# ruihuang1124/CAFE-MPC

Hardware: AMD Instinct MI355X
Metric: DDP iterations/sec, Mini-Cheetah WB N=200, batch=4096; 1/2/4/8 GPU (higher is better)
Workload: dtype f64

## Files before the change

cafe-mpc_amd/csrc/sweep.hpp:

```cpp
#pragma once
#include <cstddef>
#include <limits>
#include <type_traits>
#include "hs_types.hpp"
#include "hs_mfma.hpp"

namespace hs {

constexpr int SW_NT = 256;
constexpr int SW_SET_WB = 0, SW_SET_HKD = 1;
constexpr int SW_N = 36;
constexpr int SW_PRE = 20;
#ifndef SW_UNROLL_N
#define SW_UNROLL_N 4
#endif
#define HS_STR_(x) #x
#define HS_UNROLL_N(n) _Pragma(HS_STR_(unroll n))
#ifndef SW_LDLT_NB
#define SW_LDLT_NB ((M <= 12 || sizeof(R) == 4) ? 2 : 1)
#endif
#ifndef SW_MINB
#define SW_MINB 2
#endif
#ifndef SW_LDLT_WDW
#define SW_LDLT_WDW 1
#endif
#ifndef SW_OVERLAP_LDLT
#define SW_OVERLAP_LDLT 1
#endif

template <int N, int M, int PY, class R = double> struct SweepLdsT {
    static constexpr int LDN = N + 1, LDM = (M > PY ? M : PY) + 1, PYd = PY > 0 ? PY : 1;
    static constexpr int AR = rec_arows(N), LDA = AR + 1, A0 = N - AR;
    R H[LDN * N], A[LDA * N], HA[LDN * N];
    R B[LDA * M], HB[LDN * M];
    R Qux[LDM * N];
    union { R K[LDM * N]; R lC[PY > 0 ? LDM * N : 1]; };
    R C[PY > 0 ? LDM * N : 1], D[PY > 0 ? LDM * M : 1];
    union { R LQ[LDM * M]; R lD[PY > 0 ? LDM * M : 1]; };
    R lyy[PY > 0 ? LDM * PY : 1], Quu[LDM * M];
    R G[N], Gn[N], Qx[N], Qu[M], dU[M], ly[PYd], def[N];
};
template <int N, int M, int PY, class R = double> struct LinLdsT {
    static constexpr int AR = rec_arows(N), A0 = N - AR;
    R A[2][AR * N], Q[2][N * N], B[2][AR * M], K[2][M * N], U[2][M * M], v[2][256];
    R dx[N], dxn[N], du[M];
};
struct SweepCtl { double dV1, dV2, xfer[SW_N]; unsigned long long t_last; int ok; };
constexpr size_t sw_max(size_t a, size_t b) { return a > b ? a : b; }
template <class R> constexpr size_t sweep_bytes_wb() { return sw_max(sw_max(sizeof(SweepLdsT<36, 12, 12, R>), sizeof(LinLdsT<36, 12, 12, R>)), sw_max(sizeof(SweepLdsT<12, 12, 0, R>), sizeof(LinLdsT<12, 12, 0, R>))); }
template <class R> constexpr size_t sweep_bytes_hkd() { return sw_max(sw_max(sizeof(SweepLdsT<24, 24, 0, R>), sizeof(LinLdsT<24, 24, 0, R>)), sw_max(sizeof(SweepLdsT<12, 12, 0, R>), sizeof(LinLdsT<12, 12, 0, R>))); }
template <class R, int SET> struct SweepLdsRaw { R raw[(SET == 0 ? sweep_bytes_wb<R>() : sweep_bytes_hkd<R>()) / sizeof(R)]; SweepCtl c; };
using SweepLds = SweepLdsRaw<double, 0>;
using SweepLdsHkd = SweepLdsRaw<double, 1>;
using SweepLds32 = SweepLdsRaw<float, 1>;

#define CM(M, i, j, ld) (M)[(i) + (ld) * (j)]

#if defined(SW_PROF) && !defined(HS_HOST_EMU)
__device__ unsigned long long g_sw_prof[48];
#define SW_STAMP(i) { if (blockIdx.x == 0 && threadIdx.x == 0) { unsigned long long t_ = clock64(); atomicAdd(&g_sw_prof[i], t_ - SWC.t_last); SWC.t_last = t_; } }
#define SW_STAMP0() { if (blockIdx.x == 0 && threadIdx.x == 0) SWC.t_last = clock64(); }
#define SW_WSTAMP(p) { if (blockIdx.x == 0 && (tid & 63) == 0) atomicAdd(&g_sw_prof[16 + 4 * (p) + (tid >> 6)], clock64() - SWC.t_last); }
#else
#define SW_WSTAMP(p)
#define SW_STAMP(i)
#define SW_STAMP0()
#endif

#ifdef HS_HOST_EMU
#define SW_PRE_DECL static R pre_all_[SW_NT][SW_PRE];
#define PRE(r) pre_all_[tid][r]
#else
#define SW_PRE_DECL R pre_[SW_PRE];
#define PRE(r) pre_[r]
#endif

#ifndef HS_HOST_EMU
template <int CTRL> HD double dpp_quad(double v) {
    const int lo = __builtin_amdgcn_mov_dpp(__double2loint(v), CTRL, 0xf, 0xf, true), hi = __builtin_amdgcn_mov_dpp(__double2hiint(v), CTRL, 0xf, 0xf, true);
    return __hiloint2double(hi, lo);
}
HD double quad_sum(double v) { v += dpp_quad<0xB1>(v); v += dpp_quad<0x4E>(v); return v; }
template <int CTRL> HD float dpp_quad(float v) { return __int_as_float(__builtin_amdgcn_mov_dpp(__float_as_int(v), CTRL, 0xf, 0xf, true)); }
HD float quad_sum(float v) { v += dpp_quad<0xB1>(v); v += dpp_quad<0x4E>(v); return v; }
#endif
#ifdef HS_HOST_EMU
#define SW_QS 1
#define SW_QUAD_ROWS(CNT, PARTIAL, FINISH) if (tid < (CNT)) { const int o = tid; R p_[4]; R p2_[4]; for (int part = 0; part < 4; part++) { R partial = 0; R partial2 = 0; PARTIAL p_[part] = partial; p2_[part] = partial2; } \
    const R total = (p_[0] + p_[1]) + (p_[2] + p_[3]); const R total2 = (p2_[0] + p2_[1]) + (p2_[2] + p2_[3]); (void)total2; FINISH }
#else
#define SW_QS 4
#define SW_QUAD_ROWS(CNT, PARTIAL, FINISH) if ((tid >> 2) < (CNT)) { const int o = tid >> 2; const int part = tid & 3; R partial = 0; R partial2 = 0; PARTIAL \
    const R total = quad_sum(partial); const R total2 = quad_sum(partial2); (void)total2; if (part == 0) FINISH }
#endif

template <int M, int LD, class R, int PART>
HD void ldlt_parts(int tid, const R* A, R diag_add, R* NI, R* Lw, int* iw, int* ok, R* W1 = nullptr, R* W2 = nullptr) {
    const R TOL = R(1.0) / std::numeric_limits<R>::max();
#ifdef HS_HOST_EMU
    if (PART == 2) return;
    if (tid == 0) {
        R m[M * M]; int tr[M]; int sign = 0; (void)Lw; (void)iw;
        for (int j = 0; j < M; j++) for (int i = 0; i < M; i++) m[i + M * j] = A[i + LD * j] + (i == j ? diag_add : 0.0);
        auto Mx = [&](int i, int j) -> R& { return m[i + M * j]; };
        R temp[M];
        for (int k = 0; k < M; k++) {
            int big = k; R best = std::fabs(Mx(k, k));
            for (int i = k + 1; i < M; i++) if (std::fabs(Mx(i, i)) > best) { best = std::fabs(Mx(i, i)); big = i; }
            tr[k] = big;
            if (k != big) {
                for (int j = 0; j < k; j++) { const R t = Mx(k, j); Mx(k, j) = Mx(big, j); Mx(big, j) = t; }
                for (int i = big + 1; i < M; i++) { const R t = Mx(i, k); Mx(i, k) = Mx(i, big); Mx(i, big) = t; }
                { const R t = Mx(k, k); Mx(k, k) = Mx(big, big); Mx(big, big) = t; }
                for (int i = k + 1; i < big; i++) { const R t = Mx(i, k); Mx(i, k) = Mx(big, i); Mx(big, i) = t; }
            }
            for (int j = 0; j < k; j++) temp[j] = Mx(j, j) * Mx(k, j);
            { R s = 0; for (int j = 0; j < k; j++) s += Mx(k, j) * temp[j]; Mx(k, k) -= s; }
            for (int i = k + 1; i < M; i++) { R t = 0; for (int j = 0; j < k; j++) t += Mx(i, j) * temp[j]; Mx(i, k) -= t; }
            const R akk = Mx(k, k); const bool valid = std::fabs(akk) > 0.0;
            if (valid) for (int i = k + 1; i < M; i++) Mx(i, k) /= akk;
            if (sign == 1) { if (akk < 0) sign = 2; } else if (sign == -1) { if (akk > 0) sign = 2; } else if (sign == 0) { if (akk > 0) sign = 1; else if (akk < 0) sign = -1; }
        }
        if (!(sign == 1 || sign == 0)) *ok = 0;
        for (int c = 0; c < M; c++) {
            R x[M]; for (int i = 0; i < M; i++) x[i] = (i == c) ? 1.0 : 0.0;
            for (int k = 0; k < M; k++) if (tr[k] != k) { const R t = x[k]; x[k] = x[tr[k]]; x[tr[k]] = t; }
            for (int i = 0; i < M; i++) { R s = x[i]; for (int j = 0; j < i; j++) s -= Mx(i, j) * x[j]; x[i] = s; }
            for (int i = 0; i < M; i++) { const R d = Mx(i, i); x[i] = (std::fabs(d) > TOL) ? x[i] / d : 0.0; }
            for (int i = M - 1; i >= 0; i--) { R s = x[i]; for (int j = i + 1; j < M; j++) s -= Mx(j, i) * x[j]; x[i] = s; }
            for (int k = M - 1; k >= 0; k--) if (tr[k] != k) { const R t = x[k]; x[k] = x[tr[k]]; x[tr[k]] = t; }
            for (int i = 0; i < M; i++) NI[i + LD * c] = -x[i];
        }
    }
#else
    static_assert(M <= 32, "one row per lane");
#if defined(SW_PROF)
#define SW_LSTAMP(i) { if (blockIdx.x == 0 && tid == 0) { const unsigned long long t_ = clock64(); atomicAdd(&g_sw_prof[i], t_ - tl_); tl_ = t_; } }
#else
#define SW_LSTAMP(i)
#endif
    {
#if defined(SW_PROF)
        unsigned long long tl_ = clock64();
#endif
        const bool act = tid < M; const int me = act ? tid : M - 1;
        if (PART != 2) {
        R dg[M];
        _Pragma("unroll") for (int j = 0; j < M; j++) dg[j] = fabs(A[j + LD * j] + diag_add);
        const R mine = fabs(A[me + LD * me] + diag_add);
        int rank = 0; bool tie = false;
        _Pragma("unroll") for (int j = 0; j < M; j++) { const bool eq = (dg[j] == mine) && (j != me); rank += (dg[j] > mine || (eq && j < me)) ? 1 : 0; tie = tie || eq; }
        if (__builtin_amdgcn_ballot_w64(tie && act) == 0ull) { if (act) iw[rank] = me; }
        else {
            int gt = 0, ge = 0;
            _Pragma("unroll") for (int j = 0; j < M; j++) { gt += (dg[j] > mine) ? 1 : 0; ge += (dg[j] >= mine) ? 1 : 0; }
            int ixp = me; if (!act) { gt = M; ge = M; }
            _Pragma("unroll") for (int k = 0; k < M; k++) {
                const unsigned long long at = __builtin_amdgcn_ballot_w64(tid >= k && gt <= k && k < ge);
                const int big = (int)__builtin_ctzll(at);
                if (big != k) {
                    const int ik = __builtin_amdgcn_readlane(ixp, k), gk = __builtin_amdgcn_readlane(gt, k), ek = __builtin_amdgcn_readlane(ge, k);
                    const int ib = __builtin_amdgcn_readlane(ixp, big), gb = __builtin_amdgcn_readlane(gt, big), eb = __builtin_amdgcn_readlane(ge, big);
                    ixp = (tid == k) ? ib : ((tid == big) ? ik : ixp); gt = (tid == k) ? gb : ((tid == big) ? gk : gt); ge = (tid == k) ? eb : ((tid == big) ? ek : ge);
                }
            }
            if (act) iw[tid] = ixp;
        }
        __builtin_amdgcn_fence(__ATOMIC_RELEASE, "wavefront"); __builtin_amdgcn_wave_barrier(); __builtin_amdgcn_fence(__ATOMIC_ACQUIRE, "wavefront");
        SW_LSTAMP(9)
        }
        int pv[M]; int myrank = 0;
        _Pragma("unroll") for (int k = 0; k < M; k++) { pv[k] = iw[k]; myrank = (pv[k] == me) ? k : myrank; }
        if (PART != 2) {
        const int prow = iw[me];
        R arow[M];
        _Pragma("unroll") for (int j = 0; j < M; j++) { const int r = prow > pv[j] ? prow : pv[j], c = prow > pv[j] ? pv[j] : prow; arow[j] = A[r + LD * c] + ((j == me) ? diag_add : 0.0); }
        SW_LSTAMP(10)
        bool anyneg = false;
        _Pragma("unroll") for (int j = 0; j < M; j++) {
            const R d = hs_readlane(arow[j], j);
            R rd = hs_rcp(d); rd = rd * (R(2.0) - d * rd); rd = rd * (R(2.0) - d * rd);
            rd = (fabs(d) > TOL) ? rd : 0.0;
            anyneg = anyneg || (d < 0.0);
            const R lij = (fabs(d) > 0.0) ? arow[j] * rd : arow[j];
            if (M <= 12) { if (act && me >= j) Lw[me * M + j] = (me == j) ? rd : lij; }
            else if (act) { if (me > j) Lw[me * M + j] = lij; else if (me == j) Lw[j * M + j] = rd; }
            _Pragma("unroll") for (int k = j + 1; k < M; k++) arow[k] -= lij * hs_readlane(arow[j], k);
        }
        SW_LSTAMP(11)
        if (tid == 0 && anyneg) *ok = 0;
        }
        if (PART == 1) return;
        __builtin_amdgcn_fence(__ATOMIC_RELEASE, "wavefront"); __builtin_amdgcn_wave_barrier(); __builtin_amdgcn_fence(__ATOMIC_ACQUIRE, "wavefront");
        constexpr int NB = SW_LDLT_NB;
        R y[M], lr[NB][M];
        if (NB == 1) { lr[0][0] = 0.0; }
        _Pragma("unroll") for (int k = 0; k < M; k++) {
            if (NB == 2) { if (k + 1 < M) { _Pragma("unroll") for (int j = 0; j <= k; j++) lr[(k + 1) % NB][j] = Lw[(k + 1) * M + j]; } }
            else { _Pragma("unroll") for (int j = 0; j < k; j++) lr[0][j] = Lw[k * M + j]; }
            HS_CBAR();
            R sacc = (k == myrank) ? 1.0 : 0.0;
            _Pragma("unroll") for (int j = 0; j < k; j++) sacc -= lr[k % NB][j] * y[j];
            HS_PIN(sacc);
            y[k] = sacc;
        }
        SW_LSTAMP(12)
#if SW_LDLT_WDW
        if (PART == 2 && sizeof(R) == 8) {
            if (act) { _Pragma("unroll") for (int k = 0; k < M; k++) { W1[k + M * me] = y[k]; W2[k + M * me] = -(y[k] * Lw[k * M + k]); } }
            __builtin_amdgcn_fence(__ATOMIC_RELEASE, "wavefront"); __builtin_amdgcn_wave_barrier(); __builtin_amdgcn_fence(__ATOMIC_ACQUIRE, "wavefront");
            constexpr int TMq = (M + 15) / 16;
            MTileT<R> td[TMq * TMq];
            _Pragma("unroll") for (int t = 0; t < TMq * TMq; t++) td[t] = MTileT<R>{NI, LD, nullptr, 0, 16 * (t % TMq), 16 * (t / TMq), M, M, W1, M, W2, M, M, true, nullptr, 0, nullptr, 0, 0};
            mfma_tiles<TMq * TMq, (M + 3) / 4 * 4, 0, R>(tid, td);
            SW_LSTAMP(13)
            return;
        }
#endif
        _Pragma("unroll") for (int k = 0; k < M; k++) y[k] = y[k] * Lw[k * M + k];
        _Pragma("unroll") for (int k = M - 1; k >= 0; k--) {
            if (NB == 2) { if (k > 0) { _Pragma("unroll") for (int j = k; j < M; j++) lr[(k - 1) % NB][j] = Lw[j * M + (k - 1)]; } }
            else { _Pragma("unroll") for (int j = k + 1; j < M; j++) lr[0][j] = Lw[j * M + k]; }
            HS_CBAR();
            R sacc = y[k];
            _Pragma("unroll") for (int j = k + 1; j < M; j++) sacc -= lr[k % NB][j] * y[j];
            HS_PIN(sacc);
            y[k] = sacc;
        }
        if (act) { _Pragma("unroll") for (int k = 0; k < M; k++) NI[pv[k] + LD * me] = -y[k]; }
        SW_LSTAMP(13)
    }
#endif
}
template <int M, int LD, class R>
HD void ldlt_inverse_w(const R* A, R diag_add, R* NI, R* Lw, int* iw, int* ok) {
    HS_WPHASE(ldlt_parts<M, LD, R, 0>(tid, A, diag_add, NI, Lw, iw, ok);)
}
template <int NT, class TD, class TS> HD void ld_mat(int tid, TD* dst, int ldd, const TS* src, int rows, int cols) {
    const int i = tid % rows, j0 = tid / rows, js = NT / rows;
    if (j0 < js) for (int j = j0; j < cols; j += js) dst[i + ldd * j] = src[i + rows * j];
}
template <int NT, class TD, class TS> HD void st_mat(int tid, TD* dst, const TS* src, int lds_, int rows, int cols) {
    const int i = tid % rows, j0 = tid / rows, js = NT / rows;
    if (j0 < js) for (int j = j0; j < cols; j += js) dst[i + rows * j] = src[i + lds_ * j];
}

#define SW_RICCATI_FETCH(kk_, k_) { \
    const HS_GLOBAL R* rec_ = grec + (kk_) * (size_t)RL::size + tid; \
    _Pragma("unroll") for (int r = 0; r < RL::rounds; r++) if (r < RL::rA || r >= RL::rA + RL::rQ) PRE(r) = rec_[NT * r];      \
    PRE(RL::rounds) = (tid < N + M + PY) ? rec_[RL::oLx] : (tid < 2 * N + M + PY) ? (R)gDefect[((size_t)b * (h + 1) + (k_) + 1) * N + tid - N - M - PY] : R(0.0); }
#define SW_RICCATI_FETCH_LXX(kk_) { \
    const HS_GLOBAL R* rec_ = grec + (kk_) * (size_t)RL::size + tid; \
    _Pragma("unroll") for (int r = RL::rA; r < RL::rA + RL::rQ; r++) PRE(r) = rec_[NT * r]; }
#define SW_RICCATI_LXX() { \
    _Pragma("unroll") for (int r = 0; r < RL::rQ; r++) { const int e = tid + NT * r; if (e < N * N) S.H[(e % N) + LDN * (e / N)] += PRE(RL::rA + r); } }
#define SW_RICCATI_COMMIT() { \
    constexpr int PYd = PY > 0 ? PY : 1; \
    _Pragma("unroll") for (int r = 0; r < RL::rA; r++) { const int e = tid + NT * r; if (e < AR * N) S.A[(e % AR) + LDA * (e / AR)] = PRE(r); } \
    _Pragma("unroll") for (int r = 0; r < RL::rB; r++) { const int e = tid + NT * r; if (e < AR * M) S.B[(e % AR) + LDA * (e / AR)] = PRE(RL::rA + RL::rQ + r); } \
    _Pragma("unroll") for (int r = 0; r < RL::rC; r++) { const int e = tid + NT * r; if (e < PY * N) S.C[(e % PYd) + LDM * (e / PYd)] = PRE(RL::rA + RL::rQ + RL::rB + r); } \
    _Pragma("unroll") for (int r = 0; r < RL::rD; r++) { const int e = tid + NT * r; if (e < PY * M) S.D[(e % PYd) + LDM * (e / PYd)] = PRE(RL::rA + RL::rQ + RL::rB + RL::rC + r); } \
    _Pragma("unroll") for (int r = 0; r < RL::rLuu; r++) { const int e = tid + NT * r; if (e < M * M) S.Quu[(e % M) + LDM * (e / M)] = PRE(RL::rA + RL::rQ + RL::rB + RL::rC + RL::rD + r); } \
    _Pragma("unroll") for (int r = 0; r < RL::rLyy; r++) { const int e = tid + NT * r; if (e < PY * PY) S.lyy[(e % PYd) + LDM * (e / PYd)] = PRE(RL::rA + RL::rQ + RL::rB + RL::rC + RL::rD + RL::rLuu + r); } \
    if (tid < N) S.Qx[tid] = PRE(RL::rounds); else if (tid < N + M) S.Qu[tid - N] = PRE(RL::rounds); else if (tid < N + M + PY) S.ly[tid - N - M] = PRE(RL::rounds); \
    else if (tid < 2 * N + M + PY) S.def[tid - N - M - PY] = PRE(RL::rounds); }

template <class R> HD const HS_GLOBAL R* rec_of(const PhaseDev& P);
template <> HD const HS_GLOBAL double* rec_of<double>(const PhaseDev& P) { return P.rec; }
template <> HD const HS_GLOBAL float* rec_of<float>(const PhaseDev& P) { return P.rec32; }

template <class E> HD constexpr int deal_order(int n, int ix) {
    int c = 0;
    for (int e = 0; e < n; e++) if (!E::edge(e)) { if (c == ix) return e; c++; }
    for (int e = 0; e < n; e++) if (E::edge(e)) { if (c == ix) return e; c++; }
    return ix;
}
template <int W, int N, int M, int PY, class R, int DEAL = 0>
HD void sweep_tiles1(SweepLdsT<N, M, PY, R>& S, int lane, R dt) {
    constexpr int LDN = SweepLdsT<N, M, PY, R>::LDN, LDM = SweepLdsT<N, M, PY, R>::LDM, AR = SweepLdsT<N, M, PY, R>::AR, LDA = SweepLdsT<N, M, PY, R>::LDA, A0 = SweepLdsT<N, M, PY, R>::A0;
    constexpr int TN = (N + 15) / 16, TM = (M + 15) / 16, TP = (PY + 15) / 16, TPd = TP > 0 ? TP : 1;
    constexpr int t1 = TN * TN, t2 = t1 + TN * TM, t3 = t2 + TP * TN, t4 = t3 + TP * TM;
    constexpr bool WBT = (DEAL == 0 && t4 == 16 && t3 == 15);
    constexpr int nA = t1 + (t3 - t2), nB = (t2 - t1) + (t4 - t3);
    constexpr int NTL = DEAL == 1 ? (W == 0 ? nB : (nA - (W - 1) + 2) / 3) : WBT ? (W == 0 ? 5 : W == 3 ? 3 : 4) : (t4 - W + 3) / 4;
    if (NTL <= 0) return;
    MTileT<R> td[NTL > 0 ? NTL : 1];
    _Pragma("unroll") for (int q = 0; q < NTL; q++) {
        struct E1 { static constexpr bool edge(int e) { return e < t1 ? mfma_edge_tile<R>(N, N, 16 * (e % TN), 16 * (e / TN)) : mfma_edge_tile<R>(PY, N, 16 * ((e - t1) % TPd), 16 * ((e - t1) / TPd)); } };
        const int ix = DEAL == 1 && W > 0 ? deal_order<E1>(nA, (W - 1) + 3 * q) : (W - 1) + 3 * q;
        const int t = DEAL == 1 ? (W == 0 ? (q < t2 - t1 ? t1 + q : t3 + (q - (t2 - t1))) : (ix < t1 ? ix : t2 + (ix - t1))) : (WBT && W == 0 && q == 4) ? 15 : W + 4 * q;
        if (t < t1) { td[q] = MTileT<R>{S.HA, LDN, nullptr, 0, 16 * (t % TN), 16 * (t / TN), N, N, S.H + LDN * A0, LDN, S.A, LDA, AR, false, nullptr, 0, nullptr, 0, 0};
                      if (A0 > 0) { td[q].T = S.H; td[q].ldt = LDN; td[q].tmode = 1; td[q].tsplit = A0; td[q].tscale = dt; } }
        else if (t < t2) td[q] = MTileT<R>{S.HB, LDN, nullptr, 0, 16 * ((t - t1) % TN), 16 * ((t - t1) / TN), N, M, S.H + LDN * A0, LDN, S.B, LDA, AR, false, nullptr, 0, nullptr, 0, 0};
        else if (t < t3) td[q] = MTileT<R>{S.lC, LDM, nullptr, 0, 16 * ((t - t2) % TPd), 16 * ((t - t2) / TPd), PY, N, S.lyy, LDM, S.C, LDM, PY, false, nullptr, 0, nullptr, 0, 0};
        else td[q] = MTileT<R>{S.lD, LDM, nullptr, 0, 16 * ((t - t3) % TPd), 16 * ((t - t3) / TPd), PY, M, S.lyy, LDM, S.D, LDM, PY, false, nullptr, 0, nullptr, 0, 0};
    }
    mfma_tiles<(NTL > 0 ? NTL : 1), ((AR > PY ? AR : PY) + 3) / 4 * 4, 0, R>(lane, td);
}
template <int W, int N, int M, int PY, class R, int DEAL = 0>
HD void sweep_tiles2(SweepLdsT<N, M, PY, R>& S, int lane, R reg, R dt) {
    constexpr int LDN = SweepLdsT<N, M, PY, R>::LDN, LDM = SweepLdsT<N, M, PY, R>::LDM, AR = SweepLdsT<N, M, PY, R>::AR, LDA = SweepLdsT<N, M, PY, R>::LDA, A0 = SweepLdsT<N, M, PY, R>::A0;
    constexpr int TN = (N + 15) / 16, TM = (M + 15) / 16;
    constexpr int t1 = TN * (TN + 1) / 2, t2 = t1 + TM * TN, t3 = t2 + TM * TM;
    constexpr int NTL = DEAL == 0 ? (t3 - W + 3) / 4 : DEAL == 2 ? (t3 - t2 - W + 3) / 4 : (W == 0 ? t3 - t2 : (t2 - (W - 1) + 2) / 3);
    if (NTL <= 0) return;
    MTileT<R> td[NTL > 0 ? NTL : 1];
    _Pragma("unroll") for (int q = 0; q < NTL; q++) {
        struct E2 { static constexpr bool edge(int e) {
            if (e < t1) { int c = 0; for (int jj = 0; jj < TN; jj++) for (int ii = 0; ii <= jj; ii++) { if (c == e) return mfma_edge_tile<R>(N, N, 16 * ii, 16 * jj); c++; } return false; }
            return mfma_edge_tile<R>(M, N, 16 * ((e - t1) % TM), 16 * ((e - t1) / TM)); } };
        const int t = DEAL == 0 ? W + 4 * q : DEAL == 2 ? t2 + W + 4 * q : (W == 0 ? t2 + q : deal_order<E2>(t2, (W - 1) + 3 * q));
        int bi = 0, bj = 0;
        { int c = 0; for (int jj = 0; jj < TN; jj++) for (int ii = 0; ii <= jj; ii++) { if (c == t) { bi = ii; bj = jj; } c++; } }
        if (t < t1) { td[q] = MTileT<R>{S.H, LDN, nullptr, 0, 16 * bi, 16 * bj, N, N, S.A, LDA, S.HA + A0, LDN, AR, true, S.C, LDM, S.lC, LDM, PY}; if (bi == bj) td[q].dadd = reg; else td[q].mirror = true;
                      if (A0 > 0) { td[q].T = S.HA; td[q].ldt = LDN; td[q].tmode = 2; td[q].tsplit = A0; td[q].tscale = dt; } }
        else if (t < t2) td[q] = MTileT<R>{S.Qux, LDM, nullptr, 0, 16 * ((t - t1) % TM), 16 * ((t - t1) / TM), M, N, S.B, LDA, S.HA + A0, LDN, AR, true, S.D, LDM, S.lC, LDM, PY};
        else { td[q] = MTileT<R>{S.Quu, LDM, S.Quu, LDM, 16 * ((t - t2) % TM), 16 * ((t - t2) / TM), M, M, S.B, LDA, S.HB + A0, LDN, AR, true, S.D, LDM, S.lD, LDM, PY}; if ((t - t2) % TM == (t - t2) / TM) td[q].dadd = reg; }
    }
    mfma_tiles<(NTL > 0 ? NTL : 1), (AR + 3) / 4 * 4, (PY + 3) / 4 * 4, R>(lane, td);
}

template <int W, int N, int M, int PY, class R>
HD void sweep_tiles3(SweepLdsT<N, M, PY, R>& S, int lane) {
    constexpr int LDN = SweepLdsT<N, M, PY, R>::LDN, LDM = SweepLdsT<N, M, PY, R>::LDM;
    constexpr int TN = (N + 15) / 16;
    constexpr int NTL = (TN * TN - W + 3) / 4;
    if (NTL <= 0) return;
    MTileT<R> td[NTL > 0 ? NTL : 1];
    _Pragma("unroll") for (int q = 0; q < NTL; q++) {
        struct E3 { static constexpr bool edge(int e) { return mfma_edge_tile<R>(N, N, 16 * (e % TN), 16 * (e / TN)); } };
        const int t = deal_order<E3>(TN * TN, W + 4 * q);
        td[q] = MTileT<R>{S.H, LDN, S.H, LDN, 16 * (t % TN), 16 * (t / TN), N, N, S.Qux, LDM, S.K, LDM, M, true, nullptr, 0, nullptr, 0, 0};
    }
    mfma_tiles<(NTL > 0 ? NTL : 1), (M + 3) / 4 * 4, 0, R>(lane, td);
}

template <int W, int N, int M, int PY, class R>
HD void sweep_tilesK(SweepLdsT<N, M, PY, R>& S, int lane) {
    constexpr int LDM = SweepLdsT<N, M, PY, R>::LDM;
    constexpr int TN = (N + 15) / 16, TM = (M + 15) / 16;
    constexpr int NTL = (TM * TN - W + 3) / 4;
    if (NTL <= 0) return;
    MTileT<R> td[NTL > 0 ? NTL : 1];
    _Pragma("unroll") for (int q = 0; q < NTL; q++) {
        const int t = W + 4 * q;
        td[q] = MTileT<R>{S.K, LDM, nullptr, 0, 16 * (t % TM), 16 * (t / TM), M, N, S.LQ, LDM, S.Qux, LDM, M, false, nullptr, 0, nullptr, 0, 0};
    }
    mfma_tiles<(NTL > 0 ? NTL : 1), (M + 3) / 4 * 4, 0, R>(lane, td);
}

template <int NT, int N, int M, int PY, class R, class LDS>
HD bool riccati_phase(LDS& SS, const PhaseDev& P, int b, R reg) {
    using RL = RecLayout<N, M, PY>; using ST = SweepLdsT<N, M, PY, R>;
    static_assert(NT == 256 && RL::rounds + 1 <= SW_PRE && N <= SW_N && 2 * N + M + PY <= NT && 64 + M <= NT - N - 1 - M && N <= 64 && M <= 64, "sweep limits");
    constexpr bool WBS = (N == 36 && M == 12 && PY == 12);
    constexpr bool OVL = SW_OVERLAP_LDLT != 0;
    constexpr int GN0 = WBS ? 64 : 0, G0 = WBS ? 64 : NT - N, DV0 = WBS ? 64 + N : NT - N - 1, DU0 = WBS ? 64 + N + 1 : NT - N - 1 - M;
    constexpr int LDN = ST::LDN, LDM = ST::LDM, AR = ST::AR, LDA = ST::LDA, A0 = ST::A0;
    static_assert(sizeof(ST) <= sizeof(SS.raw), "the view fits the raw LDS block of its model set");
    ST& S = *reinterpret_cast<ST*>(SS.raw); SweepCtl& SWC = SS.c;
    constexpr int TN = (N + 15) / 16, TM = (M + 15) / 16, TP = (PY + 15) / 16;
    const int h = P.h; const R dtR = (R)P.dt;
    const auto grec = rec_of<R>(P); const auto gDefect = P.Defect; const auto gQu = P.Qu; const auto gQuu = P.Quu; const auto gQux = P.Qux;
    const auto gK = P.K; const auto gdU = P.dU; const auto gG = P.G;
    SW_PRE_DECL
    HS_PHASE(NT, { const int i = tid % N, j0 = tid / N; if (j0 < NT / N) for (int j = j0; j < N; j += NT / N) CM(S.H, i, j, LDN) += P.Phixx[(size_t)b * N * N + i + N * j]; }
             if (tid < N) { const R g = SWC.xfer[tid] + P.Phix[(size_t)b * N + tid]; S.G[tid] = g; gG[((size_t)b * (h + 1) + h) * N + tid] = g; }
             if (tid == 0) { SWC.ok = 1; }
             SW_RICCATI_FETCH((size_t)b * h + (h - 1), h - 1) SW_RICCATI_FETCH_LXX((size_t)b * h + (h - 1)))
    for (int k = h - 1; k >= 0; k--) {
        const size_t kk = (size_t)b * h + k;
        SW_STAMP0()
        HS_PHASE_L(NT, SW_RICCATI_COMMIT() if (k > 0) SW_RICCATI_FETCH(kk - 1, k - 1))
        SW_STAMP(0)
        HS_PHASE_L(NT, {
            const int w = tid >> 6, lane = tid & 63;
            if constexpr (OVL && M > 12) {
            switch (w) { case 0: sweep_tiles1<0, N, M, PY, R>(S, lane, dtR); break; case 1: sweep_tiles1<1, N, M, PY, R>(S, lane, dtR); break;
                         case 2: sweep_tiles1<2, N, M, PY, R>(S, lane, dtR); break; default: sweep_tiles1<3, N, M, PY, R>(S, lane, dtR); }
            } else if constexpr (OVL) {
            switch (w) { case 0: sweep_tiles1<0, N, M, PY, R, 1>(S, lane, dtR);
#ifndef HS_HOST_EMU
                                 __builtin_amdgcn_fence(__ATOMIC_RELEASE, "wavefront"); __builtin_amdgcn_wave_barrier(); __builtin_amdgcn_fence(__ATOMIC_ACQUIRE, "wavefront");
#endif
                                 sweep_tiles2<0, N, M, PY, R, 1>(S, lane, reg, dtR); break;
                         case 1: sweep_tiles1<1, N, M, PY, R, 1>(S, lane, dtR); break;
                         case 2: sweep_tiles1<2, N, M, PY, R, 1>(S, lane, dtR); break; default: sweep_tiles1<3, N, M, PY, R, 1>(S, lane, dtR); }
            } else {
            switch (w) { case 0: sweep_tiles1<0, N, M, PY, R>(S, lane, dtR); break; case 1: sweep_tiles1<1, N, M, PY, R>(S, lane, dtR); break;
                         case 2: sweep_tiles1<2, N, M, PY, R>(S, lane, dtR); break; default: sweep_tiles1<3, N, M, PY, R>(S, lane, dtR); }
            }
            if (tid >= GN0 && tid < GN0 + N) { const int i = tid - GN0; R s = S.G[i]; _Pragma("unroll 6") for (int j = 0; j < N; j++) s += CM(S.H, i, j, LDN) * S.def[j]; S.Gn[i] = s; }
            SW_WSTAMP(0)
        })
        if constexpr (OVL && M > 12) {
            HS_PHASE_L(NT, { const int w = tid >> 6, lane = tid & 63;
                switch (w) { case 0: sweep_tiles2<0, N, M, PY, R, 2>(S, lane, reg, dtR); break; case 1: sweep_tiles2<1, N, M, PY, R, 2>(S, lane, reg, dtR); break;
                             case 2: sweep_tiles2<2, N, M, PY, R, 2>(S, lane, reg, dtR); break; default: sweep_tiles2<3, N, M, PY, R, 2>(S, lane, reg, dtR); } })
        }
        SW_STAMP(1)
        if constexpr (OVL) {
        HS_PHASE_L(NT, {
            const int w = tid >> 6, lane = tid & 63;
            switch (w) { case 0: break; case 1: sweep_tiles2<1, N, M, PY, R, 1>(S, lane, reg, dtR); break;
                         case 2: sweep_tiles2<2, N, M, PY, R, 1>(S, lane, reg, dtR); break; default: sweep_tiles2<3, N, M, PY, R, 1>(S, lane, reg, dtR); }
            if (tid >= 128 && tid < 128 + N) {
                const int i = tid - 128; R s = 0;
                if (A0 > 0) s = (i < A0) ? S.Gn[i] : dtR * S.Gn[i - A0];
                _Pragma("unroll 6") for (int t = 0; t < AR; t++) s += CM(S.A, t, i, LDA) * S.Gn[A0 + t];
                if (PY > 0) { _Pragma("unroll 6") for (int t = 0; t < PY; t++) s += CM(S.C, t, i, LDM) * S.ly[t]; }
                S.Qx[i] += s;
            } else if (tid >= 192 && tid < 192 + M) {
                const int a = tid - 192; R s = 0;
                _Pragma("unroll 6") for (int t = 0; t < AR; t++) s += CM(S.B, t, a, LDA) * S.Gn[A0 + t];
                if (PY > 0) { _Pragma("unroll 6") for (int t = 0; t < PY; t++) s += CM(S.D, t, a, LDM) * S.ly[t]; }
                S.Qu[a] += s;
            }
            if (w == 0) ldlt_parts<M, LDM, R, 1>(lane, S.Quu, R(-1e-9), S.LQ, S.HB, reinterpret_cast<int*>(S.HB + M * M), &SWC.ok);
            SW_WSTAMP(1)
        })
        SW_STAMP(2)
        HS_PHASE_L(NT,
            if (tid < 64) ldlt_parts<M, LDM, R, 2>(tid, S.Quu, R(-1e-9), S.LQ, S.HB, reinterpret_cast<int*>(S.HB + M * M), &SWC.ok, S.HA, S.A);
            else for (int e = tid - 64; e < TN * 256; e += NT - 64) {
                const int i = 16 * (e >> 8) + (e & 15), j = 16 * (e >> 8) + ((e >> 4) & 15);
                if (i < j && j < N) { const R s = (CM(S.H, i, j, LDN) + CM(S.H, j, i, LDN)) / 2; CM(S.H, i, j, LDN) = s; CM(S.H, j, i, LDN) = s; }
            })
        SW_STAMP(5)
        } else {
        HS_PHASE_L(NT, {
            const int w = tid >> 6, lane = tid & 63;
            switch (w) { case 0: sweep_tiles2<0, N, M, PY, R>(S, lane, reg, dtR); break; case 1: sweep_tiles2<1, N, M, PY, R>(S, lane, reg, dtR); break;
                         case 2: sweep_tiles2<2, N, M, PY, R>(S, lane, reg, dtR); break; default: sweep_tiles2<3, N, M, PY, R>(S, lane, reg, dtR); }
            if (tid >= 128 && tid < 128 + N) {
                const int i = tid - 128; R s = 0;
                if (A0 > 0) s = (i < A0) ? S.Gn[i] : dtR * S.Gn[i - A0];
                _Pragma("unroll 6") for (int t = 0; t < AR; t++) s += CM(S.A, t, i, LDA) * S.Gn[A0 + t];
                if (PY > 0) { _Pragma("unroll 6") for (int t = 0; t < PY; t++) s += CM(S.C, t, i, LDM) * S.ly[t]; }
                S.Qx[i] += s;
            } else if (tid >= 192 && tid < 192 + M) {
                const int a = tid - 192; R s = 0;
                _Pragma("unroll 6") for (int t = 0; t < AR; t++) s += CM(S.B, t, a, LDA) * S.Gn[A0 + t];
                if (PY > 0) { _Pragma("unroll 6") for (int t = 0; t < PY; t++) s += CM(S.D, t, a, LDM) * S.ly[t]; }
                S.Qu[a] += s;
            }
            SW_WSTAMP(1)
        })
        SW_STAMP(2)
        HS_PHASE_L(NT, if (tid < M) gQu[kk * M + tid] = S.Qu[tid];
                   st_mat<NT>(tid, gQuu + kk * M * M, S.Quu, LDM, M, M); st_mat<NT>(tid, gQux + kk * M * N, S.Qux, LDM, M, N);)
        SW_STAMP(3)
        ldlt_inverse_w<M, LDM, R>(S.Quu, R(-1e-9), S.LQ, S.HA, reinterpret_cast<int*>(S.HB), &SWC.ok);
        SW_STAMP(4)
        HS_PHASE_L(NT,
            if (tid >= 64) for (int e = tid - 64; e < N * N; e += NT - 64) {
                const int i = e % N, j = e / N;
                if (i < j) {
                    const R s = (i / 16 == j / 16) ? (CM(S.H, i, j, LDN) + CM(S.H, j, i, LDN)) / 2 : CM(S.H, i, j, LDN);
                    CM(S.H, i, j, LDN) = s; CM(S.H, j, i, LDN) = s;
                }
            })
        SW_STAMP(5)
        }
        if (!SWC.ok) return false;
        SW_STAMP(6)
        HS_PHASE_L(NT,
            { const int w = tid >> 6, lane = tid & 63;
              switch (w) { case 0: sweep_tilesK<0, N, M, PY, R>(S, lane); break; case 1: sweep_tilesK<1, N, M, PY, R>(S, lane); break;
                           case 2: sweep_tilesK<2, N, M, PY, R>(S, lane); break; default: sweep_tilesK<3, N, M, PY, R>(S, lane); } }
            if (tid >= NT - M) { const int i = tid - (NT - M); R s = 0; _Pragma("unroll") for (int t = 0; t < M; t++) s += CM(S.LQ, i, t, LDM) * S.Qu[t]; S.dU[i] = s; }
            SW_RICCATI_LXX() if (k > 0) SW_RICCATI_FETCH_LXX(kk - 1) SW_WSTAMP(2))
        HS_PHASE_L(NT,
            { const int w = tid >> 6, lane = tid & 63;
              switch (w) { case 0: sweep_tiles3<0, N, M, PY, R>(S, lane); break; case 1: sweep_tiles3<1, N, M, PY, R>(S, lane); break;
                           case 2: sweep_tiles3<2, N, M, PY, R>(S, lane); break; default: sweep_tiles3<3, N, M, PY, R>(S, lane); } }
            if constexpr (!WBS && M > 12) {
                constexpr int CH = (M + 3) / 4;
                SW_QUAD_ROWS(N, { _Pragma("unroll") for (int jj = 0; jj < CH; jj++) { const int t = part * CH + jj; if (t < M) partial += CM(S.Qux, t, o, LDM) * S.dU[t]; } },
                             { const R s = S.Qx[o] + total; S.G[o] = s; gG[((size_t)b * (h + 1) + k) * N + o] = s; })
            }
            if ((WBS || M <= 12) && tid >= G0 && tid < G0 + N) { const int i = tid - G0; R s = S.Qx[i]; _Pragma("unroll") for (int t = 0; t < M; t++) s += CM(S.Qux, t, i, LDM) * S.dU[t]; S.G[i] = s; gG[((size_t)b * (h + 1) + k) * N + i] = s; }
            else if (tid == DV0) { R dVk = 0; _Pragma("unroll") for (int t = 0; t < M; t++) dVk -= S.Qu[t] * S.dU[t]; SWC.dV1 -= dVk; SWC.dV2 += dVk; }
            else if (tid >= DU0 && tid < DU0 + M) { const int a = tid - DU0; gdU[kk * M + a] = S.dU[a]; } SW_WSTAMP(3))
        SW_STAMP(7)
        if constexpr (OVL) {
        HS_PHASE_L(NT, st_mat<NT>(tid, gK + kk * M * N, S.K, LDM, M, N); if (tid < M) gQu[kk * M + tid] = S.Qu[tid];
                   st_mat<NT>(tid, gQuu + kk * M * M, S.Quu, LDM, M, M); st_mat<NT>(tid, gQux + kk * M * N, S.Qux, LDM, M, N);)
        } else {
        HS_PHASE_L(NT, st_mat<NT>(tid, gK + kk * M * N, S.K, LDM, M, N);)
        }
        SW_STAMP(8)
    }
    HS_PHASE(NT, if (tid < N) S.def[tid] = gDefect[((size_t)b * (h + 1)) * N + tid];)
    HS_PHASE(NT, if (tid < N) { R s = S.G[tid]; for (int j = 0; j < N; j++) s += CM(S.H, tid, j, LDN) * S.def[j]; S.Gn[tid] = s; })
    HS_PHASE(NT, if (tid < N) { SWC.xfer[tid] = S.Gn[tid]; gG[((size_t)b * (h + 1)) * N + tid] = S.Gn[tid]; }
             st_mat<NT>(tid, P.H0 + (size_t)b * N * N, S.H, LDN, N, N);)
    return true;
}

template <int NT, class R, int SET, class LDS>
HD bool riccati_sweep(LDS& S, const PhaseDev* ph, int nph, int b, R reg) {
    HS_PHASE(NT, if (tid == 0) { S.c.dV1 = 0.0; S.c.dV2 = 0.0; })
    for (int i = nph - 1; i >= 0; i--) {
        const PhaseDev& P = ph[i];
        const int n = P.n;
        if (i == nph - 1) {
            HS_PHASE(NT, for (int e = tid; e < (n + 1) * n; e += NT) S.raw[e] = 0.0; if (tid < n) S.c.xfer[tid] = 0.0;)
        } else {
            const int nn = P.next_n, ldh = nn + 1;
            R* Hn = S.raw;
            R* Px = S.raw + (n + 1) * n;
            R* HP = S.raw + 2 * (n + 1) * n;
            const auto* Pxg = P.Px + (size_t)b * nn * n;
            R gnew = 0.0;
            HS_PHASE(NT, for (int e = tid; e < nn * n; e += NT) Px[e] = Pxg[e];)
            HS_PHASE(NT,
                for (int e = tid; e < nn * n; e += NT) { const int r = e % nn, c = e / nn; R s = 0; for (int t = 0; t < nn; t++) s += Hn[r + ldh * t] * Px[t + nn * c]; HP[e] = s; }
                if (tid >= NT - n) { const int i2 = tid - (NT - n); R s = 0; for (int t = 0; t < nn; t++) s += Px[t + nn * i2] * S.c.xfer[t]; S.raw[3 * (n + 1) * n + i2] = s; })
            (void)gnew;
            HS_PHASE(NT,
                for (int e = tid; e < n * n; e += NT) { const int r = e % n, c = e / n; R s = 0; for (int t = 0; t < nn; t++) s += Px[t + nn * r] * HP[t + nn * c]; S.raw[r + (n + 1) * c] = s; }
                if (tid >= NT - n) S.c.xfer[tid - (NT - n)] = S.raw[3 * (n + 1) * n + tid - (NT - n)];)
        }
        bool ok;
        if constexpr (SET == SW_SET_WB) {
            if (P.model == HSDDP_MODEL_WB) ok = riccati_phase<NT, 36, 12, 12, R>(S, P, b, reg); else ok = riccati_phase<NT, 12, 12, 0, R>(S, P, b, reg);
        } else {
            if (P.model == HSDDP_MODEL_SRB) ok = riccati_phase<NT, 12, 12, 0, R>(S, P, b, reg); else ok = riccati_phase<NT, 24, 24, 0, R>(S, P, b, reg);
        }
        if (!ok) return false;
    }
    return true;
}

#define SW_LIN_FETCH(kk_, k_) { \
    const HS_GLOBAL R* rec_ = grec + (kk_) * (size_t)RL::size + tid; \
    _Pragma("unroll") for (int r = 0; r < RL::rA; r++) PRE(r) = rec_[RL::oA + NT * r]; \
    _Pragma("unroll") for (int r = 0; r < RL::rQ; r++) PRE(RL::rA + r) = rec_[RL::oLxx + NT * r]; \
    _Pragma("unroll") for (int r = 0; r < RL::rB; r++) PRE(RL::rA + RL::rQ + r) = rec_[RL::oB + NT * r]; \
    _Pragma("unroll") for (int r = 0; r < rK; r++) { const int e = tid + NT * r; PRE(RL::rA + RL::rQ + RL::rB + r) = (e < M * N) ? (R)gK[(kk_) * M * N + e] : R(0.0); } \
    _Pragma("unroll") for (int r = 0; r < RL::rLuu; r++) PRE(RL::rA + RL::rQ + RL::rB + rK + r) = rec_[RL::oLuu + NT * r]; \
    PRE(RL::rA + RL::rQ + RL::rB + rK + RL::rLuu) = (tid < N + M) ? rec_[RL::oLx] : (tid < N + 2 * M) ? (R)gdU[(kk_) * M + tid - N - M] \
            : (tid < 2 * N + 2 * M) ? (R)gDefect[((size_t)b * (h + 1) + (k_) + 1) * N + tid - N - 2 * M] : R(0.0); }
#define SW_LIN_COMMIT(p_) { \
    R* A_ = S.A[p_]; R* Q_ = S.Q[p_]; R* B_ = S.B[p_]; R* K_ = S.K[p_]; R* U_ = S.U[p_]; R* v_ = S.v[p_]; \
    _Pragma("unroll") for (int r = 0; r < RL::rA; r++) { const int e = tid + NT * r; if (e < AR * N) A_[e] = PRE(r); } \
    _Pragma("unroll") for (int r = 0; r < RL::rQ; r++) { const int e = tid + NT * r; if (e < N * N) Q_[e] = PRE(RL::rA + r); } \
    _Pragma("unroll") for (int r = 0; r < RL::rB; r++) { const int e = tid + NT * r; if (e < AR * M) B_[e] = PRE(RL::rA + RL::rQ + r); } \
    _Pragma("unroll") for (int r = 0; r < rK; r++) { const int e = tid + NT * r; if (e < N * M) K_[e] = PRE(RL::rA + RL::rQ + RL::rB + r); } \
    _Pragma("unroll") for (int r = 0; r < RL::rLuu; r++) { const int e = tid + NT * r; if (e < M * M) U_[e] = PRE(RL::rA + RL::rQ + RL::rB + rK + r); } \
    { const R w_ = PRE(RL::rA + RL::rQ + RL::rB + rK + RL::rLuu); \
      if (tid < N) v_[tid] = w_; else if (tid < N + M) v_[64 + tid - N] = w_; \
      else if (tid < N + 2 * M) v_[128 + tid - N - M] = w_; else if (tid < 2 * N + 2 * M) v_[192 + tid - N - 2 * M] = w_; } }

template <int NT, int N, int M, int PY, class R, class LDS>
HD void linear_phase(LDS& SS, const PhaseDev& P, int b, R eps) {
    using RL = RecLayout<N, M, PY>; using ST = LinLdsT<N, M, PY, R>;
    constexpr int rK = rec_rnd(M * N) / 256, AR = ST::AR, A0 = ST::A0;
    static_assert(RL::rA + RL::rQ + RL::rB + rK + RL::rLuu + 1 <= SW_PRE && 2 * N + 2 * M <= NT && 4 * N <= 192 && 4 * M <= NT && 192 + M <= NT && N <= 64 && M <= 64, "prefetch registers / lane maps");
    const R dtR = (R)P.dt;
    static_assert(offsetof(ST, dx) >= 2 * NT * sizeof(R), "the partial-sum scratch must not reach dx");
    static_assert(sizeof(ST) <= sizeof(SS.raw), "the view fits the raw LDS block of its model set");
    ST& S = *reinterpret_cast<ST*>(SS.raw); SweepCtl& SWC = SS.c;
    const int h = P.h;
    const auto grec = rec_of<R>(P); const auto gDefect = P.Defect; const auto gK = P.K; const auto gdU = P.dU; const auto gdX = P.dX; const auto gKdX = P.KdX;
    SW_PRE_DECL
#ifdef HS_HOST_EMU
    static R acc1_all_[NT], acc2_all_[NT];
    for (int t = 0; t < NT; t++) { acc1_all_[t] = 0.0; acc2_all_[t] = 0.0; }
#define ACC1 acc1_all_[tid]
#define ACC2 acc2_all_[tid]
#else
    R acc1_ = 0.0, acc2_ = 0.0;
#define ACC1 acc1_
#define ACC2 acc2_
#endif
    HS_PHASE(NT, if (tid < N) { R v = SWC.xfer[tid] + eps * gDefect[((size_t)b * (h + 1)) * N + tid]; S.dx[tid] = v; gdX[((size_t)b * (h + 1)) * N + tid] = v; }
             SW_LIN_FETCH((size_t)b * h, 0))
    HS_PHASE_L(NT, SW_LIN_COMMIT(0) if (1 < h) SW_LIN_FETCH((size_t)b * h + 1, 1))
    for (int k = 0; k < h; k++) {
        const size_t kk = (size_t)b * h + k;
        const int p = k & 1;
        const R* A_ = S.A[p]; const R* Q_ = S.Q[p]; const R* B_ = S.B[p]; const R* K_ = S.K[p]; const R* U_ = S.U[p];
        const R* Qx_ = S.v[p]; const R* Qu_ = S.v[p] + 64; const R* dU_ = S.v[p] + 128; const R* def_ = S.v[p] + 192;
        const R* dxc = p ? S.dxn : S.dx; R* dxw = p ? S.dx : S.dxn;
        HS_PHASE_L(NT, SW_QUAD_ROWS(M, {
            constexpr int CH = (N + 3) / 4; R s = 0;
            _Pragma("unroll") for (int jj = 0; jj < CH; jj++) { const int j = part * CH + jj; if (j < N) s += CM(K_, o, j, M) * dxc[j]; }
            partial = s; }, { S.du[o] = eps * dU_[o] + total; gKdX[kk * M + o] = total; }))
        HS_PHASE_L(NT,
            SW_QUAD_ROWS(N, {
                constexpr int T = N + M; constexpr int CH = (T + 3) / 4; constexpr int CQ = (N + 3) / 4; R s = 0; R q = 0;
                if (o >= A0) {
                    _Pragma("unroll") for (int jj = 0; jj < CH; jj++) { const int t = part * CH + jj; if (t < N) s += CM(A_, o - A0, t, AR) * dxc[t]; else if (t < T) s += CM(B_, o - A0, t - N, AR) * S.du[t - N]; }
                } else if (part == 0) s = dxc[o] + dtR * dxc[A0 + o];
                _Pragma("unroll") for (int jj = 0; jj < CQ; jj++) { const int j = part * CQ + jj; if (j < N) q += CM(Q_, o, j, N) * dxc[j]; }
                partial = s; partial2 = q; }, {
                const R v = total + eps * def_[o];
                dxw[o] = v; gdX[((size_t)b * (h + 1) + k + 1) * N + o] = v;
                ACC2 += dxc[o] * total2;
                ACC1 += Qx_[o] * dxc[o]; })
            if (tid >= 192 && tid < 192 + M) {
                const int a = tid - 192; R q = 0;
                _Pragma("unroll") for (int j = 0; j < M; j++) q += CM(U_, a, j, M) * S.du[j];
                ACC2 += S.du[a] * q; ACC1 += Qu_[a] * S.du[a];
            }
            if (k + 1 < h) { SW_LIN_COMMIT(1 - p) if (k + 2 < h) SW_LIN_FETCH(kk + 2, k + 2) })
    }
    const R* dxe = (h & 1) ? S.dxn : S.dx;
    HS_PHASE(NT, for (int e = tid; e < N * N; e += NT) S.Q[0][e] = P.Phixx[(size_t)b * N * N + e];)
    HS_PHASE(NT, if (tid % SW_QS == 0 && tid / SW_QS < N) { const int o = tid / SW_QS;
                     R q = 0; for (int j = 0; j < N; j++) q += CM(S.Q[0], o, j, N) * dxe[j]; ACC2 += dxe[o] * q; ACC1 += P.Phix[(size_t)b * N + o] * dxe[o]; })
    R* scr = SS.raw;
    HS_PHASE(NT, scr[tid] = ACC1; scr[NT + tid] = ACC2;)
    HS_PHASE(NT, if (tid == 0) { R a1 = 0, a2 = 0; for (int j = 0; j < N; j++) { a1 += scr[SW_QS * j]; a2 += scr[NT + SW_QS * j]; }
                                 R b1 = 0, b2 = 0; for (int j = 0; j < M; j++) { b1 += scr[192 + j]; b2 += scr[NT + 192 + j]; }
                                 SWC.dV1 += a1 + b1; SWC.dV2 += a2; SWC.dV2 += b2; }
             if (tid >= 64 && tid < 64 + N) SWC.xfer[tid - 64] = dxe[tid - 64];)
#undef ACC1
#undef ACC2
}

template <int NT, class R, int SET, class LDS>
HD void linear_rollout(LDS& S, const PhaseDev* ph, int nph, int b, R eps) {
    HS_PHASE(NT, if (tid == 0) { S.c.dV1 = 0.0; S.c.dV2 = 0.0; } if (tid < SW_N) S.c.xfer[tid] = 0.0;)
    for (int i = 0; i < nph; i++) {
        const PhaseDev& P = ph[i];
        if (i > 0) {
            const PhaseDev& Pp = ph[i - 1]; const int np = Pp.n, n = P.n;
            const auto* Pxg = Pp.Px + (size_t)b * n * np;
            HS_PHASE(NT, if (tid < n) { R s = 0; for (int t = 0; t < np; t++) s += Pxg[tid + n * t] * S.c.xfer[t]; S.raw[tid] = s; })
            HS_PHASE(NT, if (tid < n) S.c.xfer[tid] = S.raw[tid];)
        }
        if constexpr (SET == SW_SET_WB) {
            if (P.model == HSDDP_MODEL_WB) linear_phase<NT, 36, 12, 12, R>(S, P, b, eps); else linear_phase<NT, 12, 12, 0, R>(S, P, b, eps);
        } else {
            if (P.model == HSDDP_MODEL_SRB) linear_phase<NT, 12, 12, 0, R>(S, P, b, eps); else linear_phase<NT, 24, 24, 0, R>(S, P, b, eps);
        }
    }
}

}
```

Before: 99360.

## Add direct register-resident linear rollout phase for WB f64 model

Adds a specialized linear_phase path for the whole-body model (N=36, M=12, double). Each lane prefetches its slice of the per-knot A/B/K/Q records straight from global memory into registers, two knots ahead, instead of staging full matrices in LDS. The matvecs are split across quads of lanes and reduced with quad sums. This is meant to remove LDS commit traffic and barriers per knot, at the cost of more register pressure and much more complex lane mapping code.

```diff
diff --git a/cafe-mpc_amd/csrc/sweep.hpp b/cafe-mpc_amd/csrc/sweep.hpp
--- a/cafe-mpc_amd/csrc/sweep.hpp
+++ b/cafe-mpc_amd/csrc/sweep.hpp
@@ -554,8 +554,114 @@
       if (tid < N) v_[tid] = w_; else if (tid < N + M) v_[64 + tid - N] = w_; \
       else if (tid < N + 2 * M) v_[128 + tid - N - M] = w_; else if (tid < 2 * N + 2 * M) v_[192 + tid - N - 2 * M] = w_; } }
 
+#ifndef SW_LIN_DIRECT
+#define SW_LIN_DIRECT 1
+#endif
+#define SW_LD_UNPAREN(...) __VA_ARGS__
+template <class R> struct LinOpsT { R x[12], q[9], v0, v1, v2; };
+template <class R> struct LinDirLdsT { R Q[36 * 36]; R v[2 * 36 + 12]; };
+#ifdef HS_HOST_EMU
+#define SW_LD_DECL static LinOpsT<R> ops_all_[2][SW_NT]; static R acc1_all_[SW_NT], acc2_all_[SW_NT], qp_all_[SW_NT], qp2_all_[SW_NT]; \
+    for (int t = 0; t < SW_NT; t++) { acc1_all_[t] = 0.0; acc2_all_[t] = 0.0; }
+#define SW_LD_OPS(s_, l_) ops_all_[s_][l_]
+#define SW_LD_ACC1(l_) acc1_all_[l_]
+#define SW_LD_ACC2(l_) acc2_all_[l_]
+#define SW_LD_PHASE(...) { for (int tid = 0; tid < NT; ++tid) { SW_LD_LANE __VA_ARGS__ } }
+#define SW_LD_PHASE2(A, B) { for (int tid = 0; tid < NT; ++tid) { SW_LD_LANE SW_LD_UNPAREN A } for (int tid = 0; tid < NT; ++tid) { SW_LD_LANE SW_LD_UNPAREN B } }
+#define SW_LD_QUAD(COND, PINS, FINISH) { if (COND) { qp_all_[tid] = partial; qp2_all_[tid] = partial2; if (part == 3) { const int fl = tid - 3; \
+    const R total = (qp_all_[fl] + qp_all_[fl + 1]) + (qp_all_[fl + 2] + qp_all_[fl + 3]); const R total2 = (qp2_all_[fl] + qp2_all_[fl + 1]) + (qp2_all_[fl + 2] + qp2_all_[fl + 3]); (void)total2; FINISH } } }
+#define SW_LD_ARRIVED(s_)
+#else
+#define SW_LD_DECL LinOpsT<R> ops_[2] = {}; R acc1_ = 0.0, acc2_ = 0.0; int tid_ = threadIdx.x; asm volatile("" : "+v"(tid_)); __builtin_assume(tid_ >= 0 && tid_ < SW_NT); const int tid = tid_; SW_LD_LANE
+#define SW_LD_OPS(s_, l_) ops_[s_]
+#define SW_LD_ACC1(l_) acc1_
+#define SW_LD_ACC2(l_) acc2_
+#define SW_LD_PHASE(...) { { __VA_ARGS__ } asm volatile("s_waitcnt lgkmcnt(0)" ::: "memory"); __builtin_amdgcn_s_barrier(); asm volatile("" ::: "memory"); }
+#define SW_LD_PHASE2(A, B) SW_LD_PHASE(SW_LD_UNPAREN A SW_LD_UNPAREN B)
+#define SW_LD_QUAD(COND, PINS, FINISH) { R total = quad_sum(partial); R total2 = quad_sum(partial2); (void)total2; PINS if ((COND) && part == 0) { const int fl = tid; FINISH } }
+#define SW_LD_ARRIVED(s_) { asm volatile("" : "+v"(total)); asm volatile("" : "+v"(total2)); \
+    _Pragma("unroll") for (int jj = 0; jj < 12; jj++) asm volatile("" : "+v"(ops_[s_].x[jj])); _Pragma("unroll") for (int jj = 0; jj < 9; jj++) asm volatile("" : "+v"(ops_[s_].q[jj])); \
+    asm volatile("" : "+v"(ops_[s_].v0)); asm volatile("" : "+v"(ops_[s_].v1)); asm volatile("" : "+v"(ops_[s_].v2)); }
+#endif
+#define SW_LD_LANE const int o = tid >> 2, part = tid & 3; (void)part; \
+    const unsigned offQ = RL::oLxx + o + N * CQ * part; (void)offQ; \
+    const unsigned offX = tid >= 192 ? RL::oLuu + (tid - 192) : o < M ? o + M * CQ * part : part < 3 ? RL::oA + (o - A0) + AR * CH * part : RL::oB + (o - A0); (void)offX;
+#define SW_LD_FETCH(s_, kn_, k_) { \
+    const HS_GLOBAL R* rk_ = grec + (kn_) * (size_t)RL::size; LinOpsT<R>& F_ = SW_LD_OPS(s_, tid); \
+    if (tid < 4 * N) { \
+        if (o >= A0) { _Pragma("unroll") for (int jj = 0; jj < CH; jj++) F_.x[jj] = rk_[offX + AR * jj]; } \
+        else if (o < M) { const HS_GLOBAL double* kp_ = gK + (kn_) * (size_t)(M * N); _Pragma("unroll") for (int jj = 0; jj < CQ; jj++) F_.x[jj] = (R)kp_[offX + M * jj]; } \
+        _Pragma("unroll") for (int jj = 0; jj < CQ; jj++) F_.q[jj] = rk_[offQ + N * jj]; \
+        if (part == 0) { F_.v0 = (R)gDefect[((size_t)b * (h + 1) + (k_) + 1) * N + o]; F_.v1 = rk_[RL::oLx + o]; if (o < M) F_.v2 = (R)gdU[(kn_) * (size_t)M + o]; } \
+    } else if (tid >= 192 && tid < 192 + M) { \
+        _Pragma("unroll") for (int jj = 0; jj < M; jj++) F_.x[jj] = rk_[offX + M * jj]; \
+        F_.v1 = rk_[RL::oLu + tid - 192]; } }
+#define SW_LD_KNOT(k_, s_, xc_, xw_) { \
+    const size_t kk = (size_t)b * h + (k_); \
+     \
+    SW_LD_PHASE(if (tid < 4 * M) { \
+        const LinOpsT<R>& C_ = SW_LD_OPS(s_, tid); const R* dxc = S.v + (xc_); R partial = 0; R partial2 = 0; \
+        { R s = 0; const R* dv = dxc + CQ * part; _Pragma("unroll") for (int jj = 0; jj < CQ; jj++) s += C_.x[jj] * dv[jj]; partial = s; } \
+        SW_LD_QUAD(true, , { S.v[2 * N + o] = eps * SW_LD_OPS(s_, fl).v2 + total; gKdX[kk * M + o] = total; }) })       \
+     \
+    SW_LD_PHASE2(( \
+        const R* dxc = S.v + (xc_); R* dxw = S.v + (xw_); R partial = 0; R partial2 = 0; \
+        if (tid < 4 * N) { \
+            const LinOpsT<R>& C_ = SW_LD_OPS(s_, tid); R s = 0; R q = 0; \
+            if (o >= A0) { const R* dv = part < 3 ? dxc + CH * part : S.v + 2 * N;       \
+                _Pragma("unroll") for (int jj = 0; jj < CH; jj++) s += C_.x[jj] * dv[jj]; \
+            } else if (part == 0) s = dxc[o] + dtR * dxc[A0 + o];       \
+            { const R* dv = dxc + CQ * part; _Pragma("unroll") for (int jj = 0; jj < CQ; jj++) q += C_.q[jj] * dv[jj]; } \
+            partial = s; partial2 = q; \
+        } else if (tid >= 192 && tid < 192 + M) { \
+            const LinOpsT<R>& C_ = SW_LD_OPS(s_, tid); const R* du = S.v + 2 * N; const int a = tid - 192; R q = 0; \
+            _Pragma("unroll") for (int j = 0; j < M; j++) q += C_.x[j] * du[j]; \
+            SW_LD_ACC2(tid) += du[a] * q; SW_LD_ACC1(tid) += C_.v1 * du[a];       \
+        } \
+        SW_LD_QUAD(tid < 4 * N, SW_LD_ARRIVED(1 - (s_)), { \
+            const R v = total + eps * SW_LD_OPS(s_, fl).v0; \
+            dxw[o] = v; gdX[((size_t)b * (h + 1) + (k_) + 1) * N + o] = v; \
+            SW_LD_ACC2(fl) += dxc[o] * total2;           \
+            SW_LD_ACC1(fl) += SW_LD_OPS(s_, fl).v1 * dxc[o]; })), \
+        (if ((k_) + 2 < h) SW_LD_FETCH(s_, kk + 2, (k_) + 2))) }
+
+template <int NT, class R, class LDS>
+HD void linear_phase_direct(LDS& SS, const PhaseDev& P, int b, R eps) {
+    constexpr int N = 36, M = 12, PY = 12;
+    using RL = RecLayout<N, M, PY>; using ST = LinDirLdsT<R>;
+    constexpr int AR = rec_arows(N), A0 = N - AR, CH = (N + M) / 4, CQ = N / 4;
+    static_assert(NT == 256 && 4 * N <= 192 && 192 + M <= NT && N % CH == 0 && A0 >= M && sizeof(ST) <= sizeof(SS.raw) && N * N >= 2 * NT, "lane maps / the partial-sum scratch must not reach dx");
+    const R dtR = (R)P.dt;
+    ST& S = *reinterpret_cast<ST*>(SS.raw); SweepCtl& SWC = SS.c;
+    const int h = P.h;
+    const auto grec = rec_of<R>(P); const auto gDefect = P.Defect; const auto gK = P.K; const auto gdU = P.dU; const auto gdX = P.dX; const auto gKdX = P.KdX; const auto gPhixx = P.Phixx;
+    SW_LD_DECL
+    HS_PHASE(NT, if (tid < N) { R v = SWC.xfer[tid] + eps * gDefect[((size_t)b * (h + 1)) * N + tid]; S.v[tid] = v; gdX[((size_t)b * (h + 1)) * N + tid] = v; })
+    SW_LD_PHASE(SW_LD_FETCH(0, (size_t)b * h, 0) if (1 < h) SW_LD_FETCH(1, (size_t)b * h + 1, 1)
+                { R total = 0, total2 = 0; SW_LD_ARRIVED(0) SW_LD_ARRIVED(1) (void)total; (void)total2; })
+    int k = 0;
+    for (; k + 1 < h; k += 2) {
+        SW_LD_KNOT(k, 0, 0, N)
+        SW_LD_KNOT(k + 1, 1, N, 0)
+    }
+    if (k < h) SW_LD_KNOT(k, 0, 0, N)
+    const R* dxe = (h & 1) ? S.v + N : S.v;
+    HS_PHASE(NT, for (int e = tid; e < N * N; e += NT) S.Q[e] = gPhixx[(size_t)b * N * N + e];)
+    SW_LD_PHASE(if (part == 0 && o < N) {
+                    R q = 0; for (int j = 0; j < N; j++) q += CM(S.Q, o, j, N) * dxe[j]; SW_LD_ACC2(tid) += dxe[o] * q; SW_LD_ACC1(tid) += P.Phix[(size_t)b * N + o] * dxe[o]; })
+    R* scr = SS.raw;
+    SW_LD_PHASE(scr[tid] = SW_LD_ACC1(tid); scr[NT + tid] = SW_LD_ACC2(tid);)
+    HS_PHASE(NT, if (tid == 0) { R a1 = 0, a2 = 0; for (int j = 0; j < N; j++) { a1 += scr[4 * j]; a2 += scr[NT + 4 * j]; }
+                                 R b1 = 0, b2 = 0; for (int j = 0; j < M; j++) { b1 += scr[192 + j]; b2 += scr[NT + 192 + j]; }
+                                 SWC.dV1 += a1 + b1; SWC.dV2 += a2; SWC.dV2 += b2; }
+             if (tid >= 64 && tid < 64 + N) SWC.xfer[tid - 64] = dxe[tid - 64];)
+}
+
 template <int NT, int N, int M, int PY, class R, class LDS>
 HD void linear_phase(LDS& SS, const PhaseDev& P, int b, R eps) {
+#if SW_LIN_DIRECT
+    if constexpr (N == 36 && M == 12 && PY == 12 && std::is_same<R, double>::value) { linear_phase_direct<NT, R>(SS, P, b, eps); return; }
+#endif
     using RL = RecLayout<N, M, PY>; using ST = LinLdsT<N, M, PY, R>;
     constexpr int rK = rec_rnd(M * N) / 256, AR = ST::AR, A0 = ST::A0;
     static_assert(RL::rA + RL::rQ + RL::rB + rK + RL::rLuu + 1 <= SW_PRE && 2 * N + 2 * M <= NT && 4 * N <= 192 && 4 * M <= NT && 192 + M <= NT && N <= 64 && M <= 64, "prefetch registers / lane maps");
```

Result: no change. 100,200, median of 6 (+0.8%).
